# fkluger/vanishing_points_2017

Hardware: AMD Instinct MI355X
Metric: images/sec (LSD->CNN->EM) + horizon-AUC parity, YUD-shape, 1/2/4/8 GPU (higher is better)
Workload: dtype f32 (CNN: f32 operands / accumulation / results; conv1 multiply EXACT bf16 pieces of the f32 operands (three per operand) on the bf16 matrix cores; conv2-5, fc6 and fc7 multiply scaled fp16 PAIRS of the f32 operands (22 of 24 significand bits, three exact products per f32 product) on the fp16 matrix

## Files before the change

### __graft_entry__.py

```python
import os
import subprocess
import sys

ROOT = os.path.dirname(os.path.abspath(__file__))
if ROOT not in sys.path:
    sys.path.insert(0, ROOT)


def build():
    from vanishing_points_2017_amd import build as vbuild
    so = vbuild.build(verbose=True)
    sim = os.path.join(ROOT, "tests", "hostsim")
    out = os.path.join(sim, "_build")
    os.makedirs(out, exist_ok=True)
    subprocess.check_call(["g++", "-O2", "-std=c++17", "-ffp-contract=off", "-fPIC", "-shared",
                           "-Wno-unknown-pragmas", os.path.join(sim, "sim_em.cpp"), "-o",
                           os.path.join(out, "libvpk_hostsim.so")])
    subprocess.check_call(["g++", "-O2", "-std=c++17", "-ffp-contract=off", "-fPIC", "-shared",
                           os.path.join(sim, "sim_raster.cpp"), "-o", os.path.join(out, "libvpk_hostsim_raster.so")])
    subprocess.check_call(["g++", "-O2", "-std=c++17", "-Wall", "-Werror", "-fPIC", "-shared",
                           os.path.join(sim, "sim_cnn_plan.cpp"), "-o", os.path.join(out, "libvpk_hostsim_cnn_plan.so")])
    odir = os.path.join(ROOT, "oracle", "_build")
    os.makedirs(odir, exist_ok=True)
    subprocess.check_call(["gcc", "-O2", "-fPIC", "-shared", "-ffp-contract=off", "-fno-builtin",
                           os.path.join(ROOT, "oracle", "_fma.c"), "-o", os.path.join(odir, "libvpkfma.so"), "-lm"])
    import vanishing_points_2017_amd
    from vanishing_points_2017_amd import _lib
    lib = _lib.load()
    missing = [s for s in _lib.EXPORTS if not hasattr(lib, s)]
    if missing:
        raise RuntimeError("libvpk.so lacks symbols: %s" % missing)
    print("built", so)


def smoke():
    import numpy as np
    import torch
    assert torch.cuda.is_available(), "smoke() needs cuda:0"
    from vanishing_points_2017_amd import synth, vp_localisation
    from oracle import em_numpy
    from oracle import agg_raster
    from vanishing_points_2017_amd import sphere_mapping
    sc = synth.make_scene(4242, 90, 3)
    ln = sc["l"]
    sc["sphere_image"] = sphere_mapping.sphere_line_plot(ln.copy(), 500, alpha=0.1)
    assert np.array_equal(sc["sphere_image"], agg_raster.raster(ln)), "the sphere raster differs from the oracle"
    got = vp_localisation.expectation_maximisation(sc["l"].copy(), sc["lp"].copy(), sc["cnn_response"],
                                                   sphere_image=sc["sphere_image"])
    ref = em_numpy.expectation_maximisation(sc["l"].copy(), sc["lp"].copy(), sc["cnn_response"].copy(),
                                            sphere_image=sc["sphere_image"])
    assert np.array_equal(got["vp_assoc"], ref["vp_assoc"]), "line->VP assignments differ from the oracle"
    assert np.abs(got["vp"] - ref["vp"]).max() < 1e-4
    from oracle import cnn_torch
    from vanishing_points_2017_amd import cnn
    w, mean = cnn.synthetic_weights(0), cnn.synthetic_mean(0)
    sphere = sc["sphere_image"][None]
    want = cnn_torch.forward(w, mean, sphere)
    net = cnn.Net(w, mean)
    err = []
    for alg in (4, 2):
        net.set_algorithm(alg)
        err.append(float(np.abs(net.forward(sphere) - want).max()))
    net.set_algorithm(4)
    assert max(err) <= 2e-5, "CNN response differs from the oracle: %s" % err
    print("smoke ok: raster of %d lines exact; %d VPs, %d iterations; CNN max |diff| %.1e (default: fp16 pairs) / %.1e (exact bf16 triples + Winograd f32)" % (
        ln.shape[0], got["vp"].shape[0], got["iterations"], err[0], err[1]))


if __name__ == "__main__":
    build()
    if len(sys.argv) > 1 and sys.argv[1] == "smoke":
        smoke()
```

### vanishing_points_2017_amd/csrc/cnn_dense_pieces.hpp

```cpp
#ifndef VPK_CNN_DENSE_PIECES_HPP_
#define VPK_CNN_DENSE_PIECES_HPP_

namespace {

constexpr int DP_THREADS = 512;
constexpr int DP_BM = 256, DP_BN = 128;
constexpr int DP_CHUNK = 32;
template <int NP> constexpr int DP_STAGE = NP * 2 * 4 * 1024;
constexpr int DP_NST = 3;
constexpr int DP_FOLD = 8;

struct DenseDims {
    int N, K, OC;
    int chunks, kparts, cpp;
    int mtiles, ntiles;
    float wscale, oscale;
    const int* live = nullptr;
};

template <int NP>
__global__ __launch_bounds__(256) void dense_split_kernel(const float* __restrict__ x, unsigned short* __restrict__ out, int N, int K,
                                                          int chunks, float ascale, unsigned* __restrict__ range_word, unsigned range_bit,
                                                          unsigned* __restrict__ img_range, const int* __restrict__ live) {
    const int c = blockIdx.x, nt = blockIdx.y;
    if (live) {
        N = __builtin_amdgcn_readfirstlane(*live);
        if (nt * DP_BN >= N) return;
    }
    const int j = threadIdx.x >> 6, lane = threadIdx.x & 63;
    const int n = nt * DP_BN + 32 * j + (lane & 31), h = lane >> 5;
    float v[16];
    if (n < N) {
        const f32x4v* src = reinterpret_cast<const f32x4v*>(x + (size_t)n * K + (size_t)c * DP_CHUNK + 16 * h);
#pragma unroll
        for (int q = 0; q < 4; ++q) {
            const f32x4v t = src[q];
            v[4 * q] = t[0]; v[4 * q + 1] = t[1]; v[4 * q + 2] = t[2]; v[4 * q + 3] = t[3];
        }
    } else {
#pragma unroll
        for (int e = 0; e < 16; ++e) v[e] = 0.f;
    }
    unsigned short p[3][16];
    bool bad = false;
#pragma unroll
    for (int e = 0; e < 16; ++e) {
        if (NP == 3) split3(v[e], p[0][e], p[1][e], p[2][e]);
        else split2h_guard(v[e] * ascale, p[0][e], p[1][e], bad);
    }
    if (NP == 2) {
        const unsigned long long m = __builtin_amdgcn_ballot_w64(bad);
        if (m != 0ull) {
            if (lane == 0) atomicOr(range_word, range_bit);
            if (img_range && lane < 32 && (((m | (m >> 32)) >> lane) & 1ull)) atomicOr(img_range + n, range_bit);
        }
    }
    u32x4* dst = reinterpret_cast<u32x4*>(out + ((size_t)nt * chunks + c) * (DP_STAGE<NP> / 2));
#pragma unroll
    for (int q = 0; q < NP; ++q)
#pragma unroll
        for (int s = 0; s < 2; ++s) {
            u32x4 w4;
#pragma unroll
            for (int e = 0; e < 4; ++e) w4[e] = (unsigned)p[q][8 * s + 2 * e] | ((unsigned)p[q][8 * s + 2 * e + 1] << 16);
            dst[(((q * 2 + s) * 4 + j) * 64) + lane] = w4;
        }
}

__global__ void dense_tile_weights_kernel(const float* __restrict__ w, float* __restrict__ out, int OC, int K, int chunks, long long total4) {
    const long long o4 = (long long)blockIdx.x * blockDim.x + threadIdx.x;
    if (o4 >= total4) return;
    const int kk4 = (int)(o4 % (DP_CHUNK / 4));
    const int r = (int)((o4 / (DP_CHUNK / 4)) % DP_BM);
    const long long tc = o4 / ((DP_CHUNK / 4) * DP_BM);
    const int c = (int)(tc % chunks);
    const int mt = (int)(tc / chunks);
    const int row = mt * DP_BM + r;
    f32x4v v = {0.f, 0.f, 0.f, 0.f};
    if (row < OC) v = *reinterpret_cast<const f32x4v*>(w + (size_t)row * K + (size_t)c * DP_CHUNK + 4 * kk4);
    reinterpret_cast<f32x4v*>(out)[o4] = v;
}

__global__ void dense_pair_weights_kernel(const float* __restrict__ w, unsigned short* __restrict__ out, int OC, int K, int chunks,
                                          float wscale, long long total16) {
    const long long o = (long long)blockIdx.x * blockDim.x + threadIdx.x;
    if (o >= total16) return;
    const int lane = (int)(o & 63);
    const int q = (int)((o >> 6) & 1), s_ = (int)((o >> 7) & 1), wv = (int)((o >> 8) & 7);
    const long long tc = o >> 11;
    const int c = (int)(tc % chunks), mt = (int)(tc / chunks);
    const int row = mt * DP_BM + 32 * wv + (lane & 31), h = lane >> 5;
    unsigned short p[8];
#pragma unroll
    for (int e = 0; e < 8; ++e) {
        const float x = row < OC ? w[(size_t)row * K + (size_t)c * DP_CHUNK + 16 * h + 8 * s_ + e] * wscale : 0.f;
        unsigned short h0, h1;
        split2h(x, h0, h1);
        p[e] = q == 0 ? h0 : h1;
    }
    u32x4 w4;
#pragma unroll
    for (int e = 0; e < 4; ++e) w4[e] = (unsigned)p[2 * e] | ((unsigned)p[2 * e + 1] << 16);
    reinterpret_cast<u32x4*>(out)[o] = w4;
}

__global__ __launch_bounds__(DP_THREADS, 2) void dense_pairs_kernel(DenseDims d, const unsigned short* __restrict__ wpair,
                                                                    const unsigned short* __restrict__ xfrag, float* __restrict__ part,
                                                                    int* __restrict__ item_counter, int total_items) {
    constexpr int NP = 2;
    __shared__ __attribute__((aligned(16))) unsigned char dp_lds[DP_NST * DP_STAGE<NP>];
    __shared__ int s_next[2];
    const int tid = threadIdx.x, lane = tid & 63;
    const int wave = __builtin_amdgcn_readfirstlane(tid >> 6);
    const int r31 = lane & 31, h = lane >> 5;
    const unsigned lds0 = lds_addr(dp_lds);
    typedef __attribute__((address_space(3))) const bf16x8 lds_cbf8;
    int parity = 0;
    for (int item = blockIdx.x; item < total_items;) {
        int nx = 0;
        if (tid == 0)
            asm volatile("s_nop 4\n\tglobal_atomic_add %0, %1, %2, %3 sc0" : "=v"(nx) : "v"(0), "v"(1), "s"(item_counter) : "memory");
        int t = item;
        const int mt = t % d.mtiles; t /= d.mtiles;
        const int nt = t % d.ntiles;
        const int ks = t / d.ntiles;
        const int c0 = ks * d.cpp, c1 = c0 + d.cpp < d.chunks ? c0 + d.cpp : d.chunks;
        const bf16x8* wbase = reinterpret_cast<const bf16x8*>(wpair) + ((size_t)mt * d.chunks * 8 + wave) * 256 + lane;
        const unsigned char* xsrc = reinterpret_cast<const unsigned char*>(xfrag) + (size_t)nt * d.chunks * DP_STAGE<NP>;
        bf16x8 af[3][2][NP];
        auto load_a = [&](int c, auto o_tag) {
            constexpr int o = decltype(o_tag)::value;
            const bf16x8* src = wbase + (size_t)c * (8 * 256);
#pragma unroll
            for (int s = 0; s < 2; ++s)
#pragma unroll
                for (int q = 0; q < NP; ++q) af[o][s][q] = src[(2 * s + q) * 64];
        };
        auto issue_b = [&](int c) {
            const unsigned char* src = xsrc + (size_t)c * DP_STAGE<NP>;
            const unsigned dst = lds0 + (unsigned)((c % DP_NST) * DP_STAGE<NP>);
#pragma unroll
            for (int k = 0; k < NP; ++k) {
                const int f = NP * wave + k;
                dma16((unsigned)(f * 1024 + lane * 16), src, __builtin_amdgcn_readfirstlane(dst + (unsigned)f * 1024u));
            }
        };
        f32x16 acc[4], tq[4];
#pragma unroll
        for (int j = 0; j < 4; ++j)
#pragma unroll
            for (int e = 0; e < 16; ++e) { acc[j][e] = 0.f; tq[j][e] = 0.f; }
        __builtin_amdgcn_s_barrier();
        load_a(c0, std::integral_constant<int, 0>());
        issue_b(c0);
        if (c0 + 1 < c1) { load_a(c0 + 1, std::integral_constant<int, 1>()); issue_b(c0 + 1); }
        int fold = 0;
        auto chunk = [&](auto o_tag, auto o2_tag, int c) {
            constexpr int o = decltype(o_tag)::value;
            if (c + 1 < c1) asm volatile("s_waitcnt vmcnt(%0)" ::"n"(4 + NP) : "memory"); else asm volatile("s_waitcnt vmcnt(0)" ::: "memory");
            if (c == c0 && tid == 0) { asm volatile("" : "+v"(nx)); s_next[parity] = nx + (int)gridDim.x; }
            __builtin_amdgcn_s_barrier();
            if (c + 2 < c1) { load_a(c + 2, o2_tag); issue_b(c + 2); }
            const unsigned stage = lds0 + (unsigned)((c % DP_NST) * DP_STAGE<NP> + lane * 16);
#pragma unroll
            for (int s = 0; s < 2; ++s) {
                bf16x8 bfr[4][NP];
#pragma unroll
                for (int j = 0; j < 4; ++j)
#pragma unroll
                    for (int q = 0; q < NP; ++q) bfr[j][q] = *(lds_cbf8*)(stage + (unsigned)((((q * 2 + s) * 4) + j) * 1024));
                constexpr int PA[3] = {1, 0, 0}, PB[3] = {0, 1, 0};
#pragma unroll
                for (int pr = 0; pr < 3; ++pr)
#pragma unroll
                    for (int j = 0; j < 4; ++j)
                        tq[j] = __builtin_amdgcn_mfma_f32_32x32x16_f16(__builtin_bit_cast(f16x8, af[o][s][PA[pr]]),
                                                                       __builtin_bit_cast(f16x8, bfr[j][PB[pr]]), tq[j], 0, 0, 0);
            }
            if (++fold == DP_FOLD || c + 1 == c1) {
#pragma unroll
                for (int j = 0; j < 4; ++j) {
                    acc[j] += tq[j];
#pragma unroll
                    for (int e = 0; e < 16; ++e) tq[j][e] = 0.f;
                }
                fold = 0;
            }
        };
        int c = c0;
        for (; c + 2 < c1; c += 3) {
            chunk(std::integral_constant<int, 0>(), std::integral_constant<int, 2>(), c);
            chunk(std::integral_constant<int, 1>(), std::integral_constant<int, 0>(), c + 1);
            chunk(std::integral_constant<int, 2>(), std::integral_constant<int, 1>(), c + 2);
        }
        if (c < c1) chunk(std::integral_constant<int, 0>(), std::integral_constant<int, 2>(), c);
        if (c + 1 < c1) chunk(std::integral_constant<int, 1>(), std::integral_constant<int, 0>(), c + 1);
#pragma unroll
        for (int j = 0; j < 4; ++j) {
            const int n = nt * DP_BN + 32 * j + r31;
            if (n >= d.N) continue;
            float* prow = part + ((size_t)ks * d.N + n) * d.OC + mt * DP_BM + 32 * wave + 4 * h;
#pragma unroll
            for (int q = 0; q < 4; ++q) {
                if (mt * DP_BM + 32 * wave + 8 * q >= d.OC) continue;
                f32x4v v4 = {acc[j][4 * q] * d.oscale, acc[j][4 * q + 1] * d.oscale, acc[j][4 * q + 2] * d.oscale, acc[j][4 * q + 3] * d.oscale};
                *reinterpret_cast<f32x4v*>(prow + 8 * q) = v4;
            }
        }
        item = __builtin_amdgcn_readfirstlane(s_next[parity]);
        parity ^= 1;
    }
}

template <int NP>
__global__ __launch_bounds__(DP_THREADS, 2) void dense_pieces_kernel(DenseDims d, const float* __restrict__ w,
                                                                     const unsigned short* __restrict__ xfrag, float* __restrict__ part,
                                                                     int* __restrict__ item_counter, int total_items) {
    __shared__ __attribute__((aligned(16))) unsigned char dp_lds[DP_NST * DP_STAGE<NP>];
    __shared__ int s_next[2];
// ... 127 lines not shown
```

### vanishing_points_2017_amd/csrc/cnn_norm_pool.hpp

```cpp
#ifndef VPK_CNN_NORM_POOL_HPP_
#define VPK_CNN_NORM_POOL_HPP_

namespace {

template <typename Px>
__global__ void prep_input_kernel(const Px* __restrict__ sphere, const float* __restrict__ mean,
                                  float* __restrict__ out, int plane) {
    const int p = blockIdx.x * blockDim.x + threadIdx.x;
    if (p >= plane) return;
    const size_t img = (size_t)blockIdx.y * plane;
    const int y = p / 500, x = p - y * 500;
    const int q = ((y % C1_PH) * C1_PH + (x % C1_PH)) * (C1_PW * C1_PW) + (y / C1_PH) * C1_PW + x / C1_PH;
    out[img + q] = (float)sphere[img + p] - mean[p];
}

constexpr int LRN_CCH = 16;
template <int TPH, int CB>
__global__ __launch_bounds__(256) void lrn5_pool3s2_stream_kernel(const float* __restrict__ in, float* __restrict__ out, int C,
                                                                  int H, int W, int PH, int PW, float alpha, float beta,
                                                                  int PHp, int PWp, int opad, int cgroups, const int* __restrict__ live) {
    constexpr int TR = 2 * TPH + 1, SLOTS = 4, PMAX = 256 * SLOTS;
    __shared__ float plane[2][CB][PMAX];
    const int tiles_h = (PH + TPH - 1) / TPH;
    const int th = blockIdx.x % tiles_h, cgi = (blockIdx.x / tiles_h) % cgroups, b = blockIdx.x / (tiles_h * cgroups);
// ... 80 lines not shown
                }
            out[((size_t)b * C + c) * PHp * PWp + (size_t)(ph + opad) * PWp + ox + opad] = m;
        }
        buf ^= 1;
    }
}

template <int TPH, int TPW>
__global__ __launch_bounds__(256) void lrn5_pool3s2_tiled_kernel(const float* __restrict__ in, float* __restrict__ out,
                                                                 int C, int H, int W, int PH, int PW, float alpha,
                                                                 float beta, int PHp, int PWp, int opad) {
    constexpr int CC = LRN_CCH, NPL = CC + 4;
    constexpr int TR = 2 * TPH + 1, TC = 2 * TPW + 1, NPIX = TR * TC;
    __shared__ float patch[NPL][NPIX];
    const int tiles_w = (PW + TPW - 1) / TPW, tiles_h = (PH + TPH - 1) / TPH;
    const int nch = (C + CC - 1) / CC;
    int bid = blockIdx.x;
    const int tw = bid % tiles_w; bid /= tiles_w;
    const int th = bid % tiles_h; bid /= tiles_h;
    const int ch = bid % nch;
    const int b = bid / nch;
    const int c0 = ch * CC;
    const int ph0 = th * TPH, pw0 = tw * TPW;
    const int h0 = 2 * ph0, w0 = 2 * pw0;
    const int HW = H * W;
    const float* x = in + (size_t)b * C * HW;
    constexpr int LU = 8;
    for (int e0 = threadIdx.x; e0 < NPL * NPIX; e0 += 256 * LU) {
        float v[LU];
#pragma unroll
        for (int u = 0; u < LU; ++u) {
            const int e = e0 + u * 256;
            const int pl = e / NPIX, p = e - pl * NPIX;
            const int r = p / TC, q = p - r * TC;
            const int c = c0 - 2 + pl, h = h0 + r, w = w0 + q;
            v[u] = 0.f;
            if (e < NPL * NPIX && c >= 0 && c < C && h < H && w < W) v[u] = x[(size_t)c * HW + (size_t)h * W + w];
        }
#pragma unroll
        for (int u = 0; u < LU; ++u) {
            const int e = e0 + u * 256;
            if (e < NPL * NPIX) patch[0][e] = v[u];
        }
    }
    __syncthreads();
    const float an = alpha / 5.f;
    for (int p = threadIdx.x; p < NPIX; p += 256) {
        float v0 = patch[0][p], v1 = patch[1][p], v2 = patch[2][p], v3 = patch[3][p];
#pragma unroll
        for (int k = 0; k < CC; ++k) {
            const float v4 = patch[k + 4][p];
            const float sc = 1.f + an * (v0 * v0 + v1 * v1 + v2 * v2 + v3 * v3 + v4 * v4);
            float pw_;
            if (beta == 0.75f) {
                const float r = __builtin_amdgcn_rsqf(sc);
                pw_ = r * __builtin_amdgcn_sqrtf(r);
            }
            else pw_ = powf(sc, -beta);
            patch[k + 2][p] = v2 * pw_;
            v0 = v1; v1 = v2; v2 = v3; v3 = v4;
        }
    }
    __syncthreads();
    for (int e = threadIdx.x; e < CC * TPH * TPW; e += 256) {
        const int k = e / (TPH * TPW), o = e - k * (TPH * TPW);
        const int oy = o / TPW, ox = o - oy * TPW;
        const int ph = ph0 + oy, pw = pw0 + ox, c = c0 + k;
        if (ph >= PH || pw >= PW || c >= C) continue;
        float m = -3.402823466e38f;
#pragma unroll
        for (int dy = 0; dy < 3; ++dy)
#pragma unroll
            for (int dx = 0; dx < 3; ++dx) {
                const int r = 2 * oy + dy, q = 2 * ox + dx;
                if (h0 + r < H && w0 + q < W) {
                    const float v = patch[k + 2][r * TC + q];
                    m = v > m ? v : m;
                }
            }
        out[((size_t)b * C + c) * PHp * PWp + (size_t)(ph + opad) * PWp + pw + opad] = m;
    }
}

template <int PL>
__global__ __launch_bounds__(256) void pool5_kernel(const float* __restrict__ in, float* __restrict__ out, long long planes,
                                                    const int* __restrict__ live) {
    constexpr int H = 30, W = 30, P = 15, HW = H * W, PP = P * P;
    __shared__ __attribute__((aligned(16))) float s[PL * HW];
    const long long p0 = (long long)blockIdx.x * PL;
    if (live && p0 >= (long long)*live * 256) return;
    const int np = planes - p0 < PL ? (int)(planes - p0) : PL;
    const f32x4* src = reinterpret_cast<const f32x4*>(in + p0 * HW);
    for (int q = threadIdx.x; q < np * HW / 4; q += 256) reinterpret_cast<f32x4*>(s)[q] = src[q];
    __syncthreads();
    float* dst = out + p0 * PP;
    for (int e = threadIdx.x; e < np * PP; e += 256) {
        const int pl = e / PP, o = e - pl * PP;
        const int py = o / P, px = o - py * P;
        const float* x = s + pl * HW + (2 * py) * W + 2 * px;
        const bool by = 2 * py + 2 < H, bx = 2 * px + 2 < W;
        float m = fmaxf(fmaxf(x[0], x[1]), fmaxf(x[W], x[W + 1]));
        if (bx) m = fmaxf(m, fmaxf(x[2], x[W + 2]));
        if (by) m = fmaxf(m, fmaxf(x[2 * W], x[2 * W + 1]));
        if (bx && by) m = fmaxf(m, x[2 * W + 2]);
        dst[e] = m;
    }
}

__global__ void unpad_kernel(const float* __restrict__ in, float* __restrict__ out, long long planes, int H, int W,
                             int Hp, int Wp, int pad) {
    long long idx = (long long)blockIdx.x * blockDim.x + threadIdx.x;
    if (idx >= planes * H * W) return;
    const int w = (int)(idx % W), hh = (int)((idx / W) % H);
    const long long pl = idx / ((long long)W * H);
    out[idx] = in[((size_t)pl * Hp + hh + pad) * Wp + w + pad];
}

}
#endif
```

### vanishing_points_2017_amd/csrc/cnn_plan.hpp

```cpp
#ifndef VPK_CNN_PLAN_HPP_
#define VPK_CNN_PLAN_HPP_

#include "../../include/vpk.h"

struct CnnConfig {
    int precision = 0;
    int split_variant = 0;
    int algorithm = 4;
    int fusion = 3;
    int conv1_group = 4;
    int dense_presplit = 1;
    bool profiling = false;
};

inline void cnn_config_set_precision(CnnConfig& c, int mode) {
    c.precision = mode ? 1 : 0;
    c.split_variant = mode > 1 ? mode - 1 : 0;
}

enum class Conv1Impl { GEMM, DIRECT_F32, GEMM_FUSED, PIECES3, PIECES2 };
enum class ConvImpl { DMA_F32, SPLIT_GEMM, WINOGRAD, PIECES3, PIECES2 };
enum class DenseImpl { DMA_F32, PIECES3, PIECES2_STREAMED, PIECES2_PRESPLIT };

struct ConvStage {
    ConvImpl impl = ConvImpl::DMA_F32;
    int split_tiling = 0;
    bool chained_in = false;
    bool chained_out = false;
    bool needs_to_planes = false;
    bool writes_next_planes = false;
};

struct CnnPlan {
    int err = VPK_OK;
    const char* msg = nullptr;
    bool prep_input = false;
    Conv1Impl conv1 = Conv1Impl::PIECES3;
    bool conv1_hands_planes = false;
    ConvStage conv[4];
    bool norm2_planes = false;
    bool norm2_hands_planes = false;
    DenseImpl fc[3] = {DenseImpl::DMA_F32, DenseImpl::DMA_F32, DenseImpl::DMA_F32};
};

inline CnnPlan cnn_resolve_plan(const CnnConfig& c, int tap, bool f32_images, bool device_counted) {
    CnnPlan p;
    const bool f32_mfma = c.precision == 0;
    const bool pairs = f32_mfma && c.algorithm == 4;
    const bool triples = f32_mfma && c.algorithm >= 2 && !pairs;
    const bool wino = f32_mfma && c.algorithm >= 1;
    const bool split = c.precision == 1;

    if (tap == 0 || c.fusion == 0) p.conv1 = Conv1Impl::GEMM;
    else if (c.fusion == 1) p.conv1 = Conv1Impl::DIRECT_F32;
    else if (c.fusion == 2) p.conv1 = Conv1Impl::GEMM_FUSED;
    else p.conv1 = c.fusion == 4 ? Conv1Impl::PIECES2 : Conv1Impl::PIECES3;
    p.prep_input = p.conv1 == Conv1Impl::GEMM || p.conv1 == Conv1Impl::GEMM_FUSED;
    const bool conv1_pieces = p.conv1 == Conv1Impl::PIECES3 || p.conv1 == Conv1Impl::PIECES2;
    p.conv1_hands_planes = conv1_pieces && pairs && tap != 1;
    if (f32_images && p.conv1 == Conv1Impl::PIECES2) {
        p.err = VPK_ERR_STATE;
        p.msg = "vpk_cnn_forward_f32: vpk_cnn_set_fusion(4) takes uint8 rasters only";
    }

    const ConvImpl pieces = pairs ? ConvImpl::PIECES2 : ConvImpl::PIECES3;
    const ConvImpl other = split ? ConvImpl::SPLIT_GEMM : (wino ? ConvImpl::WINOGRAD : ConvImpl::DMA_F32);
    const bool pieces35 = pairs || (triples && c.algorithm == 3);
    p.conv[0].impl = pairs || triples ? pieces : other;
    p.conv[1].impl = pieces35 ? pieces : other;
    p.conv[2].impl = pairs ? pieces : other;
    p.conv[3].impl = pieces35 ? pieces : other;
    p.norm2_planes = pairs;
    p.norm2_hands_planes = pairs && tap != 3;
    p.conv[1].writes_next_planes = pairs && tap != 4;
    p.conv[2].writes_next_planes = pairs && tap != 5;
    p.conv[0].needs_to_planes = (pairs || triples) && !p.conv1_hands_planes;
    p.conv[1].needs_to_planes = pieces35 && !p.norm2_hands_planes;
    p.conv[2].needs_to_planes = pairs && !p.conv[1].writes_next_planes;
    p.conv[3].needs_to_planes = pieces35 && !p.conv[2].writes_next_planes;
    const bool chain = split && tap != 4 && tap != 5;
    p.conv[1].chained_out = p.conv[2].chained_in = p.conv[2].chained_out = p.conv[3].chained_in = chain;
    for (int i = 0; i < 4; ++i) p.conv[i].split_tiling = c.split_variant == 0 ? (i <= 1 ? 1 : 0) : c.split_variant - 1;

    const DenseImpl dense2 = c.dense_presplit ? DenseImpl::PIECES2_PRESPLIT : DenseImpl::PIECES2_STREAMED;
    if (pairs) p.fc[0] = p.fc[1] = dense2;
    else if (triples) p.fc[0] = DenseImpl::PIECES3;

    if (device_counted) {
        const bool counted = p.conv1 == Conv1Impl::PIECES3 && p.conv[0].impl == ConvImpl::PIECES3 &&
                             p.conv[1].impl == ConvImpl::WINOGRAD && p.conv[2].impl == ConvImpl::WINOGRAD &&
                             p.conv[3].impl == ConvImpl::WINOGRAD && !p.norm2_planes && p.fc[0] == DenseImpl::PIECES3 &&
                             p.fc[1] == DenseImpl::DMA_F32 && p.fc[2] == DenseImpl::DMA_F32 && tap < 0 && !c.profiling;
        if (!counted) {
            p.err = VPK_ERR_STATE;
            p.msg = "run_forward: a device-counted pass runs algorithm 2 with the default conv1, untapped";
        }
    }
    return p;
}

#endif
```

### vanishing_points_2017_amd/csrc/vpk_cnn.hip

```cpp
#include "vpk_internal.hpp"

#include <stdlib.h>
#include <string.h>
#include <type_traits>
#include <vector>

#include "cnn_plan.hpp"
#include "cnn_topology.hpp"
#include "cnn_gemm_f32.hpp"
#include "cnn_conv1_direct.hpp"
#include "cnn_norm_pool.hpp"

namespace {

#include "cnn_split_gemm.hpp"
#include "cnn_pairs.hpp"
#include "cnn_conv1_pieces.hpp"
#include "cnn_conv_pieces.hpp"
#include "cnn_norm_pool_planes.hpp"
#include "cnn_dense_pieces.hpp"
#include "cnn_winograd.hpp"

struct Layer {
    ConvDims d;
// ... 243 lines not shown
                               S->L[1].wino, S->L[1].bias, dst, ctr + 1, total);
            return;
        }
        WinoDims wd = S->L[li].wd;
        wd.tiles = batch * WG_TILES_PER_IMAGE;
        const int total = wd.groups * wd.ocblocks * ((wd.tiles + WG_TB - 1) / WG_TB);
        hipLaunchKernelGGL(conv3x3_winograd_kernel, dim3((unsigned)std::min(total, h->num_cu)), dim3(WG_THREADS), 0, st, wd, src,
                           S->L[li].wino, S->L[li].bias, dst, ctr + li, total, live);
    };
    auto to_p6 = [&](int li, bool pairs, const float* src, unsigned short* dst) {
        const ConvDims& d = S->L[li].d;
        const int C = d.IC * d.groups;
        if (pairs) hipLaunchKernelGGL(to_planes_kernel<2>, dim3((unsigned)d.Hp, (unsigned)(C / 16), (unsigned)batch), dim3(256), 0, st, src, dst, C, d.Hp, d.Wp,
                                      S->L[li].ascale, fc.range_word, 1u << li, fc.img_range, live);
        else hipLaunchKernelGGL(to_planes_kernel<3>, dim3((unsigned)d.Hp, (unsigned)(C / 16), (unsigned)batch), dim3(256), 0, st, src, dst, C, d.Hp, d.Wp, 1.f,
                                fc.range_word, 0u, nullptr, live);
    };
    auto conv_pieces = [&](int li, bool pairs, const unsigned short* src6, float* dst, unsigned short* planes_next) {
        PieceDims pd = pairs ? S->L[li].pdh : S->L[li].pd;
        pd.B = batch;
        if (planes_next) { const PieceDims& nx = S->L[li + 1].pdh; pd.o_cgtot = nx.CGtot; pd.o_Hp = nx.Hp; pd.o_Wp = nx.Wp; pd.o_pad = 1; pd.o_ascale = S->L[li + 1].ascale; }
        pd.range_word = fc.range_word; pd.range_bit = 1u << (li + 1); pd.img_range = fc.img_range; pd.live = live;
        if (pairs) pd.oscale = 1.f / (S->L[li].hscale * S->L[li].ascale);
        constexpr int nb = 4;
        const int tile_rows = pairs && li == 3 ? 2 * nb : nb;
        pd.rtiles = (pd.OH + tile_rows - 1) / tile_rows;
        const int total = pd.groups * batch * pd.rtiles * pd.ctiles * pd.mtiles;
        const unsigned blocks = (unsigned)std::min(total, 2 * h->num_cu);
        auto go = [&](auto kernel) {
            hipLaunchKernelGGL(kernel, dim3(blocks), dim3(CP_THREADS), 0, st, pd, src6, pairs ? S->L[li].whalf : S->L[li].wsplit, S->L[li].bias,
                               dst, planes_next, ctr + li, total);
        };
        if (pairs) { if (li == 1) go(conv_pieces_kernel<5, nb, 2, 1>); else if (li == 3) go(conv_pieces_kernel<3, nb, 2, 2>); else go(conv_pieces_kernel<3, nb, 2, 1>); }
        else { if (li == 1) go(conv_pieces_kernel<5, nb, 3, 1>); else go(conv_pieces_kernel<3, nb, 3, 1>); }
    };
    auto conv_stage = [&](int li, const float* src, float* dst, unsigned short* planes, unsigned short* planes_next,
                          const unsigned short* split_in, unsigned short* split_out) {
        const ConvStage& cs = plan.conv[li - 1];
        const bool pairs = cs.impl == ConvImpl::PIECES2;
        switch (cs.impl) {
        case ConvImpl::PIECES3:
        case ConvImpl::PIECES2:
            if (cs.needs_to_planes) to_p6(li, pairs, src, planes);
            conv_pieces(li, pairs, planes, dst, cs.writes_next_planes ? planes_next : nullptr);
            break;
        case ConvImpl::SPLIT_GEMM:
            conv_split(li, cs.split_tiling, src, cs.chained_in ? split_in : nullptr, cs.chained_out ? (void*)split_out : (void*)dst, cs.chained_out);
            break;
        case ConvImpl::WINOGRAD:
            conv_wino(li, src, dst);
            break;
        case ConvImpl::DMA_F32:
            if (li == 3) launch_dma(h, conv_gemm_dma_kernel<1, 4, 3, 1, false>, dims(3), 96, src, S->L[3], dst, 1, ctr + 3);
            else launch_dma(h, conv_gemm_dma_kernel<2, 2, 2, 2, false>, dims(li), 128, src, S->L[li], dst, 1, ctr + li);
            break;
        }
    };
    unsigned short* p6_2 = reinterpret_cast<unsigned short*>(R[R_P6_2]);
    unsigned short* p6_3 = reinterpret_cast<unsigned short*>(R[R_P6_3]);
    unsigned short* p6_5 = reinterpret_cast<unsigned short*>(R[R_P6_5]);
    unsigned short* s4 = reinterpret_cast<unsigned short*>(R[R_SPLIT4]);
    unsigned short* s5 = reinterpret_cast<unsigned short*>(R[R_SPLIT5]);
    conv_stage(1, R[R_POOL1], R[R_CONV2], p6_2, nullptr, nullptr, nullptr);
    mark(1);
    if ((rc = tapcopy(2, R[R_CONV2], A_CONV2))) return rc;
    if (plan.norm2_planes)
        hipLaunchKernelGGL((lrn5_pool3s2_planes_kernel<6>), dim3((unsigned)(batch * 5 * 8)), dim3(256), 0, st, R[R_CONV2], R[R_POOL2],
                           plan.norm2_hands_planes ? p6_3 : nullptr, 256, 61, 61, 30, 30, 1e-4f, 32, 32, 1, 8,
                           S->L[2].ascale, fc.range_word, 1u << 2, fc.img_range);
    else
        hipLaunchKernelGGL((lrn5_pool3s2_stream_kernel<6, 4>), dim3((unsigned)(batch * 5 * 8)), dim3(256), 0, st, R[R_CONV2], R[R_POOL2],
                           256, 61, 61, 30, 30, 1e-4f, 0.75f, 32, 32, 1, 8, live);
    mark(2);
    tapunpad(3, R[R_POOL2], 256, 30, 30, 1);
    conv_stage(2, R[R_POOL2], R[R_CONV3], p6_3, p6_5, nullptr, s4);
    mark(1);
    tapunpad(4, R[R_CONV3], 384, 30, 30, 1);
    conv_stage(3, R[R_CONV3], R[R_CONV4], p6_5, p6_3, s4, s5);
    mark(1);
    tapunpad(5, R[R_CONV4], 384, 30, 30, 1);
    conv_stage(4, R[R_CONV4], R[R_CONV5], plan.conv[2].writes_next_planes ? p6_3 : p6_5, nullptr, s5, nullptr);
    mark(1);
    if ((rc = tapcopy(6, R[R_CONV5], A_CONV5))) return rc;
    hipLaunchKernelGGL((pool5_kernel<8>), dim3((unsigned)(((long long)batch * 256 + 7) / 8)), dim3(256), 0, st, R[R_CONV5], R[R_POOL5],
                       (long long)batch * 256, live);
    mark(1);
    if ((rc = tapcopy(7, R[R_POOL5], A_POOL5))) return rc;

    float* fc_in = R[R_POOL5];
    float* fc_out = R[R_FCA];
    for (int li = 5; li < 8; ++li) {
        ConvDims d = dims(li);
        const DenseImpl impl = plan.fc[li - 5];
        if (impl == DenseImpl::DMA_F32) {
            launch_dma(h, conv_gemm_dma_kernel<2, 2, 2, 2, true>, d, 128, fc_in, S->L[li], R[R_PART], 1, ctr + li, 3, live);
        } else {
            const bool pairs = impl != DenseImpl::PIECES3;
            DenseDims dd;
            dd.N = batch; dd.K = d.K; dd.OC = d.OC; dd.chunks = d.K / DP_CHUNK;
            dd.kparts = li == 5 ? 45 : 16;
            dd.cpp = dd.chunks / dd.kparts;
            dd.mtiles = (d.OC + DP_BM - 1) / DP_BM; dd.ntiles = (batch + DP_BN - 1) / DP_BN;
            dd.wscale = pairs ? S->L[li].hscale : 1.f;
            dd.live = live;
            dd.oscale = pairs ? 1.f / (S->L[li].hscale * S->L[li].ascale) : 1.f;
            const size_t need = (size_t)dd.ntiles * (TOPO[5].IC / DP_CHUNK) * DP_STAGE<3>;
            if ((rc = vpk_reserve(h, (void**)&S->xfrag, &S->xfrag_bytes, need, "hipMalloc(dense input fragments)"))) return rc;
            const int total = dd.mtiles * dd.ntiles * dd.kparts;
            const dim3 split_grid((unsigned)dd.chunks, (unsigned)dd.ntiles), grid((unsigned)std::min(total, h->num_cu));
            if (pairs)
                hipLaunchKernelGGL(dense_split_kernel<2>, split_grid, dim3(256), 0, st, fc_in, S->xfrag, batch,
                                   d.K, dd.chunks, S->L[li].ascale, fc.range_word, 1u << li, fc.img_range, nullptr);
            else
                hipLaunchKernelGGL(dense_split_kernel<3>, split_grid, dim3(256), 0, st, fc_in, S->xfrag, batch,
                                   d.K, dd.chunks, 1.f, fc.range_word, 0u, nullptr, live);
            switch (impl) {
            case DenseImpl::PIECES2_PRESPLIT:
                hipLaunchKernelGGL(dense_pairs_kernel, grid, dim3(DP_THREADS), 0, st, dd, S->L[li].wpair, S->xfrag, R[R_PART], ctr + li, total);
                break;
            case DenseImpl::PIECES2_STREAMED:
                hipLaunchKernelGGL(dense_pieces_kernel<2>, grid, dim3(DP_THREADS), 0, st, dd, S->L[li].wraw, S->xfrag, R[R_PART], ctr + li, total);
                break;
            default:
                hipLaunchKernelGGL(dense_pieces_kernel<3>, grid, dim3(DP_THREADS), 0, st, dd, S->L[li].wraw, S->xfrag, R[R_PART], ctr + li, total);
                break;
            }
            d.ksplit = dd.kparts;
        }
        const long long tot = (long long)d.N * d.OC;
        float* dst = li == 7 ? out : fc_out;
        float* pre = (li == 7 && tap == 10) ? tap_out : nullptr;
        hipLaunchKernelGGL(splitk_reduce_kernel, dim3(ew_blocks(tot)), dim3(256), 0, st, R[R_PART], S->L[li].bias, d.ksplit,
                           d.N, d.OC, li == 7 ? 2 : 1, dst, pre, live);
        mark(1);
        if (li == 5 && (rc = tapcopy(8, fc_out, A_FC6))) return rc;
        if (li == 6 && (rc = tapcopy(9, fc_out, A_FC7))) return rc;
        fc_in = fc_out;
        fc_out = (li == 5) ? R[R_FCB] : R[R_FCA];
    }
    if (cfg.profiling) {
        S->ev_valid = (evi == 14);
        if (S->ev_valid) ++S->ev_pass;
    }
    VPK_HIP(h, hipGetLastError());
    return VPK_OK;
}

}
#include "cnn_calibrate.hpp"
#include "cnn_range_policy.hpp"

namespace {

struct ScopedDeviceBuffer {
    void* p = nullptr;
    ~ScopedDeviceBuffer() { if (p) (void)hipFree(p); }
};

template <typename T>
int upload(vpk_handle* h, T** dst, const T* src, size_t n) {
    VPK_HIP(h, hipMalloc((void**)dst, n * sizeof(T)));
    VPK_HIP(h, hipMemcpy(*dst, src, n * sizeof(T), hipMemcpyHostToDevice));
    return VPK_OK;
}

int load_model(vpk_handle* h, const float* const blobs[16], const float* mean) {
    vpk_cnn_state* S = h->cnn;
    int rc;
    if ((rc = upload(h, &S->mean, mean, (size_t)500 * 500))) return rc;
    if (const char* e = getenv("VPK_CONV1_GROUP")) { const int v = atoi(e); if (v >= 1 && v <= 64) S->cfg.conv1_group = v; }
    if (const char* e = getenv("VPK_DENSE_PRESPLIT")) S->cfg.dense_presplit = atoi(e) != 0;
    for (int li = 0; li < 8; ++li) {
        const Topo& t = TOPO[li];
        const float* w = blobs[2 * li];
        Layer& l = S->L[li];
        ConvDims& d = l.d;
        d.B = 0; d.IC = t.IC; d.Hp = t.H + 2 * t.P; d.Wp = t.W + 2 * t.P; d.OC = t.OC; d.OH = t.OH; d.OW = t.OW; d.groups = t.G;
        d.OHp = t.OH + 2 * t.OP; d.OWp = t.OW + 2 * t.OP; d.opad = t.OP;
        if (li == 0) { d.IC = C1_PH * C1_PH; d.Hp = C1_PW; d.Wp = C1_PW; }
        d.K = t.IC * t.KH * t.KH;
        d.Kp = (d.K + BK - 1) / BK * BK;
        d.Mp = (t.OC + t.BM - 1) / t.BM * t.BM;
        d.N = 0;
        d.ksplit = KSPLIT[li];
        d.relu = 1;
        const size_t w_floats = (size_t)t.G * t.OC * d.K;
        const size_t p_floats = (size_t)t.G * d.Kp * d.Mp;
        {
            ScopedDeviceBuffer rawbuf;
            VPK_HIP(h, hipMalloc(&rawbuf.p, w_floats * sizeof(float)));
            const float* raw = static_cast<const float*>(rawbuf.p);
            VPK_HIP(h, hipMemcpy(rawbuf.p, w, w_floats * sizeof(float), hipMemcpyHostToDevice));
            VPK_HIP(h, hipMalloc((void**)&l.wp, p_floats * sizeof(float)));
            hipLaunchKernelGGL(pack_weights_kernel, dim3((unsigned)((p_floats + 255) / 256)), dim3(256), 0, h->stream, raw,
                               l.wp, t.G, t.OC, d.K, d.Kp, d.Mp);
            VPK_HIP(h, hipStreamSynchronize(h->stream));
            if (li == 5 || li == 6) {
                const int chunks = d.K / DP_CHUNK, mtiles = (t.OC + DP_BM - 1) / DP_BM;
                const long long total4 = (long long)mtiles * chunks * DP_BM * (DP_CHUNK / 4);
                VPK_HIP(h, hipMalloc((void**)&l.wraw, (size_t)total4 * 16));
                hipLaunchKernelGGL(dense_tile_weights_kernel, dim3((unsigned)((total4 + 255) / 256)), dim3(256), 0, h->stream, raw, l.wraw, t.OC, d.K,
                                   chunks, total4);
                VPK_HIP(h, hipStreamSynchronize(h->stream));
                l.hscale = weight_scale_pow2(w, w_floats);
                const long long total16 = (long long)mtiles * chunks * 8 * 2 * 2 * 64;
                VPK_HIP(h, hipMalloc((void**)&l.wpair, (size_t)total16 * 16));
                hipLaunchKernelGGL(dense_pair_weights_kernel, dim3((unsigned)((total16 + 255) / 256)), dim3(256), 0, h->stream, raw, l.wpair, t.OC,
                                   d.K, chunks, l.hscale, total16);
                VPK_HIP(h, hipStreamSynchronize(h->stream));
            }
        }
        if (li < 5) {
            std::vector<unsigned> tab(d.Kp, 0u);
            for (int k = 0; k < d.K; ++k) {
                int ic = k / (t.KH * t.KH), r = k % (t.KH * t.KH), kh = r / t.KH, kw = r % t.KH;
                if (li == 0)
// ... 291 lines not shown
```

Measured before the change: 23270.

## Fuse pool5 and fc6 reduce with fp16-pair fragment packing for dense layers

Pool5 now writes the fc6 input directly as scaled fp16 pair fragments in the dense kernel's layout. The fc6 split-k reduce likewise applies bias and ReLU and emits fc7's input fragments directly. This removes the separate float round trips and dense_split launches for fc6 and fc7 on the default path. Weight fragment loads in the dense kernel also become nontemporal. The trade-off is extra index arithmetic and scattered 16-byte stores, and taps 7/8 fall back to the old path.

```diff
diff --git a/__graft_entry__.py b/__graft_entry__.py
--- a/__graft_entry__.py
+++ b/__graft_entry__.py
@@ -20,6 +20,8 @@
                            os.path.join(sim, "sim_raster.cpp"), "-o", os.path.join(out, "libvpk_hostsim_raster.so")])
     subprocess.check_call(["g++", "-O2", "-std=c++17", "-Wall", "-Werror", "-fPIC", "-shared",
                            os.path.join(sim, "sim_cnn_plan.cpp"), "-o", os.path.join(out, "libvpk_hostsim_cnn_plan.so")])
+    subprocess.check_call(["g++", "-O2", "-std=c++17", "-Wall", "-Werror", "-fPIC", "-shared",
+                           os.path.join(sim, "sim_cnn_dense_tail.cpp"), "-o", os.path.join(out, "libvpk_hostsim_cnn_dense_tail.so")])
     odir = os.path.join(ROOT, "oracle", "_build")
     os.makedirs(odir, exist_ok=True)
     subprocess.check_call(["gcc", "-O2", "-fPIC", "-shared", "-ffp-contract=off", "-fno-builtin",
diff --git a/vanishing_points_2017_amd/csrc/cnn_dense_pieces.hpp b/vanishing_points_2017_amd/csrc/cnn_dense_pieces.hpp
--- a/vanishing_points_2017_amd/csrc/cnn_dense_pieces.hpp
+++ b/vanishing_points_2017_amd/csrc/cnn_dense_pieces.hpp
@@ -65,6 +65,78 @@
             for (int e = 0; e < 4; ++e) w4[e] = (unsigned)p[q][8 * s + 2 * e] | ((unsigned)p[q][8 * s + 2 * e + 1] << 16);
             dst[(((q * 2 + s) * 4 + j) * 64) + lane] = w4;
         }
+}
+
+__device__ __forceinline__ size_t dense_frag_word(int n, int k, int q, int chunks) {
+    const int c = k / DP_CHUNK, kk = k % DP_CHUNK, h = kk >> 4, s = (kk >> 3) & 1;
+    const int nt = n / DP_BN, j = (n % DP_BN) >> 5, lane = (n & 31) + 32 * h;
+    return ((size_t)nt * chunks + c) * (DP_STAGE<2> / 16) + (size_t)(((q * 2 + s) * 4 + j) * 64 + lane);
+}
+
+constexpr int P5F_PL = 8, P5F_GROUPS = 256 / P5F_PL, P5F_K = P5F_PL * P5_PP;
+__global__ __launch_bounds__(256) void pool5_frags_kernel(const float* __restrict__ in, unsigned short* __restrict__ out, int N, float ascale,
+                                                          unsigned* __restrict__ range_word, unsigned range_bit,
+                                                          unsigned* __restrict__ img_range) {
+    static_assert(P5F_K % 8 == 0 && (256 * P5_PP) % DP_CHUNK == 0, "whole fragment words per workgroup, whole chunks per image");
+    constexpr int chunks = 256 * P5_PP / DP_CHUNK;
+    __shared__ __attribute__((aligned(16))) float s[P5F_PL * P5_HW];
+    __shared__ __attribute__((aligned(16))) unsigned short hp[2][P5F_K];
+    const int b = blockIdx.x, u = (b >> 6) * 8 + (b & 7);
+    const int pg = u % P5F_GROUPS, n = (u / P5F_GROUPS) * 8 + ((b >> 3) & 7);
+    u32x4* dst = reinterpret_cast<u32x4*>(out);
+    const int k0 = pg * P5F_K;
+    if (n >= N) {
+        const u32x4 z = {0u, 0u, 0u, 0u};
+        for (int w = threadIdx.x; w < 2 * (P5F_K / 8); w += 256) {
+            const int q = w / (P5F_K / 8), g = w - q * (P5F_K / 8);
+            dst[dense_frag_word(n, k0 + 8 * g, q, chunks)] = z;
+        }
+        return;
+    }
+    const f32x4* src = reinterpret_cast<const f32x4*>(in + ((size_t)n * 256 + (size_t)pg * P5F_PL) * P5_HW);
+    for (int q = threadIdx.x; q < P5F_PL * P5_HW / 4; q += 256) reinterpret_cast<f32x4*>(s)[q] = src[q];
+    __syncthreads();
+    bool bad = false;
+    for (int e = threadIdx.x; e < P5F_K; e += 256) {
+        const int pl = e / P5_PP, o = e - pl * P5_PP;
+        split2h_guard(pool5_window(s + pl * P5_HW, o) * ascale, hp[0][e], hp[1][e], bad);
+    }
+    range_report(bad, range_word, range_bit, img_range ? img_range + n : nullptr);
+    __syncthreads();
+    for (int w = threadIdx.x; w < 2 * (P5F_K / 8); w += 256) {
+        const int q = w / (P5F_K / 8), g = w - q * (P5F_K / 8);
+        dst[dense_frag_word(n, k0 + 8 * g, q, chunks)] = reinterpret_cast<const u32x4*>(hp[q])[g];
+    }
+}
+
+__global__ __launch_bounds__(256) void splitk_reduce_frags_kernel(const float* __restrict__ part, const float* __restrict__ bias, int ksplit,
+                                                                  int N, int OC, unsigned short* __restrict__ out, float ascale,
+                                                                  unsigned* __restrict__ range_word, unsigned range_bit,
+                                                                  unsigned* __restrict__ img_range) {
+    const int per = OC / 4;
+    const long long t = (long long)blockIdx.x * 256 + threadIdx.x;
+    const int n = (int)(t / per), m = 4 * (int)(t % per);
+    f32x4v v = {0.f, 0.f, 0.f, 0.f};
+    if (n < N) {
+        const f32x4v* p = reinterpret_cast<const f32x4v*>(part + (size_t)n * OC + m);
+        const size_t stride = (size_t)N * OC / 4;
+#pragma unroll 15
+        for (int s = 0; s < ksplit; ++s) v += p[s * stride];
+        v += *reinterpret_cast<const f32x4v*>(bias + m);
+#pragma unroll
+        for (int e = 0; e < 4; ++e) v[e] = v[e] > 0.f ? v[e] : 0.f;
+    }
+    unsigned short h0[4], h1[4];
+    bool bad = false;
+#pragma unroll
+    for (int e = 0; e < 4; ++e) split2h_guard(v[e] * ascale, h0[e], h1[e], bad);
+    range_report(bad, range_word, range_bit, img_range && n < N ? img_range + n : nullptr);
+    const unsigned hi[2] = {(unsigned)h0[0] | ((unsigned)h0[1] << 16), (unsigned)h0[2] | ((unsigned)h0[3] << 16)};
+    const unsigned lo[2] = {(unsigned)h1[0] | ((unsigned)h1[1] << 16), (unsigned)h1[2] | ((unsigned)h1[3] << 16)};
+    const bool odd = threadIdx.x & 1;
+    const unsigned r0 = (unsigned)__shfl_xor((int)(odd ? hi[0] : lo[0]), 1), r1 = (unsigned)__shfl_xor((int)(odd ? hi[1] : lo[1]), 1);
+    const u32x4 w4 = odd ? u32x4{r0, r1, lo[0], lo[1]} : u32x4{hi[0], hi[1], r0, r1};
+    reinterpret_cast<u32x4*>(out)[dense_frag_word(n, odd ? m - 4 : m, odd ? 1 : 0, OC / DP_CHUNK)] = w4;
 }
 
 __global__ void dense_tile_weights_kernel(const float* __restrict__ w, float* __restrict__ out, int OC, int K, int chunks, long long total4) {
@@ -134,7 +206,7 @@
 #pragma unroll
             for (int s = 0; s < 2; ++s)
 #pragma unroll
-                for (int q = 0; q < NP; ++q) af[o][s][q] = src[(2 * s + q) * 64];
+                for (int q = 0; q < NP; ++q) af[o][s][q] = __builtin_nontemporal_load(&src[(2 * s + q) * 64]);
         };
         auto issue_b = [&](int c) {
             const unsigned char* src = xsrc + (size_t)c * DP_STAGE<NP>;
diff --git a/vanishing_points_2017_amd/csrc/cnn_norm_pool.hpp b/vanishing_points_2017_amd/csrc/cnn_norm_pool.hpp
--- a/vanishing_points_2017_amd/csrc/cnn_norm_pool.hpp
+++ b/vanishing_points_2017_amd/csrc/cnn_norm_pool.hpp
@@ -186,10 +186,24 @@
     }
 }
 
+constexpr int P5_H = 30, P5_W = 30, P5_P = 15, P5_HW = P5_H * P5_W, P5_PP = P5_P * P5_P;
+
+__device__ __forceinline__ float pool5_window(const float* __restrict__ plane, int o) {
+    constexpr int H = P5_H, W = P5_W, P = P5_P;
+    const int py = o / P, px = o - py * P;
+    const float* x = plane + (2 * py) * W + 2 * px;
+    const bool by = 2 * py + 2 < H, bx = 2 * px + 2 < W;
+    float m = fmaxf(fmaxf(x[0], x[1]), fmaxf(x[W], x[W + 1]));
+    if (bx) m = fmaxf(m, fmaxf(x[2], x[W + 2]));
+    if (by) m = fmaxf(m, fmaxf(x[2 * W], x[2 * W + 1]));
+    if (bx && by) m = fmaxf(m, x[2 * W + 2]);
+    return m;
+}
+
 template <int PL>
 __global__ __launch_bounds__(256) void pool5_kernel(const float* __restrict__ in, float* __restrict__ out, long long planes,
                                                     const int* __restrict__ live) {
-    constexpr int H = 30, W = 30, P = 15, HW = H * W, PP = P * P;
+    constexpr int HW = P5_HW, PP = P5_PP;
     __shared__ __attribute__((aligned(16))) float s[PL * HW];
     const long long p0 = (long long)blockIdx.x * PL;
     if (live && p0 >= (long long)*live * 256) return;
@@ -200,14 +214,7 @@
     float* dst = out + p0 * PP;
     for (int e = threadIdx.x; e < np * PP; e += 256) {
         const int pl = e / PP, o = e - pl * PP;
-        const int py = o / P, px = o - py * P;
-        const float* x = s + pl * HW + (2 * py) * W + 2 * px;
-        const bool by = 2 * py + 2 < H, bx = 2 * px + 2 < W;
-        float m = fmaxf(fmaxf(x[0], x[1]), fmaxf(x[W], x[W + 1]));
-        if (bx) m = fmaxf(m, fmaxf(x[2], x[W + 2]));
-        if (by) m = fmaxf(m, fmaxf(x[2 * W], x[2 * W + 1]));
-        if (bx && by) m = fmaxf(m, x[2 * W + 2]);
-        dst[e] = m;
+        dst[e] = pool5_window(s + pl * HW, o);
     }
 }
 
diff --git a/vanishing_points_2017_amd/csrc/cnn_plan.hpp b/vanishing_points_2017_amd/csrc/cnn_plan.hpp
--- a/vanishing_points_2017_amd/csrc/cnn_plan.hpp
+++ b/vanishing_points_2017_amd/csrc/cnn_plan.hpp
@@ -41,6 +41,8 @@
     bool norm2_planes = false;
     bool norm2_hands_planes = false;
     DenseImpl fc[3] = {DenseImpl::DMA_F32, DenseImpl::DMA_F32, DenseImpl::DMA_F32};
+    bool pool5_hands_frags = false;
+    bool fc6_hands_frags = false;
 };
 
 inline CnnPlan cnn_resolve_plan(const CnnConfig& c, int tap, bool f32_images, bool device_counted) {
@@ -85,6 +87,9 @@
     const DenseImpl dense2 = c.dense_presplit ? DenseImpl::PIECES2_PRESPLIT : DenseImpl::PIECES2_STREAMED;
     if (pairs) p.fc[0] = p.fc[1] = dense2;
     else if (triples) p.fc[0] = DenseImpl::PIECES3;
+    const bool default_arithmetic = pairs && c.fusion == 3;
+    p.pool5_hands_frags = default_arithmetic && tap != 7;
+    p.fc6_hands_frags = default_arithmetic && tap != 8;
 
     if (device_counted) {
         const bool counted = p.conv1 == Conv1Impl::PIECES3 && p.conv[0].impl == ConvImpl::PIECES3 &&
diff --git a/vanishing_points_2017_amd/csrc/vpk_cnn.hip b/vanishing_points_2017_amd/csrc/vpk_cnn.hip
--- a/vanishing_points_2017_amd/csrc/vpk_cnn.hip
+++ b/vanishing_points_2017_amd/csrc/vpk_cnn.hip
@@ -349,8 +349,18 @@
     conv_stage(4, R[R_CONV4], R[R_CONV5], plan.conv[2].writes_next_planes ? p6_3 : p6_5, nullptr, s5, nullptr);
     mark(1);
     if ((rc = tapcopy(6, R[R_CONV5], A_CONV5))) return rc;
-    hipLaunchKernelGGL((pool5_kernel<8>), dim3((unsigned)(((long long)batch * 256 + 7) / 8)), dim3(256), 0, st, R[R_CONV5], R[R_POOL5],
-                       (long long)batch * 256, live);
+    const int dense_ntiles = (batch + DP_BN - 1) / DP_BN;
+    auto reserve_xfrag = [&]() {
+        const size_t need = (size_t)dense_ntiles * (TOPO[5].IC / DP_CHUNK) * DP_STAGE<3>;
+        return vpk_reserve(h, (void**)&S->xfrag, &S->xfrag_bytes, need, "hipMalloc(dense input fragments)");
+    };
+    if (plan.pool5_hands_frags) {
+        if ((rc = reserve_xfrag())) return rc;
+        hipLaunchKernelGGL(pool5_frags_kernel, dim3((unsigned)(dense_ntiles * DP_BN * P5F_GROUPS)), dim3(256), 0, st, R[R_CONV5], S->xfrag,
+                           batch, S->L[5].ascale, fc.range_word, 1u << 5, fc.img_range);
+    } else
+        hipLaunchKernelGGL((pool5_kernel<8>), dim3((unsigned)(((long long)batch * 256 + 7) / 8)), dim3(256), 0, st, R[R_CONV5], R[R_POOL5],
+                           (long long)batch * 256, live);
     mark(1);
     if ((rc = tapcopy(7, R[R_POOL5], A_POOL5))) return rc;
 
@@ -367,18 +377,18 @@
             dd.N = batch; dd.K = d.K; dd.OC = d.OC; dd.chunks = d.K / DP_CHUNK;
             dd.kparts = li == 5 ? 45 : 16;
             dd.cpp = dd.chunks / dd.kparts;
-            dd.mtiles = (d.OC + DP_BM - 1) / DP_BM; dd.ntiles = (batch + DP_BN - 1) / DP_BN;
+            dd.mtiles = (d.OC + DP_BM - 1) / DP_BM; dd.ntiles = dense_ntiles;
             dd.wscale = pairs ? S->L[li].hscale : 1.f;
             dd.live = live;
             dd.oscale = pairs ? 1.f / (S->L[li].hscale * S->L[li].ascale) : 1.f;
-            const size_t need = (size_t)dd.ntiles * (TOPO[5].IC / DP_CHUNK) * DP_STAGE<3>;
-            if ((rc = vpk_reserve(h, (void**)&S->xfrag, &S->xfrag_bytes, need, "hipMalloc(dense input fragments)"))) return rc;
+            if ((rc = reserve_xfrag())) return rc;
             const int total = dd.mtiles * dd.ntiles * dd.kparts;
             const dim3 split_grid((unsigned)dd.chunks, (unsigned)dd.ntiles), grid((unsigned)std::min(total, h->num_cu));
-            if (pairs)
+            const bool handed = (li == 5 && plan.pool5_hands_frags) || (li == 6 && plan.fc6_hands_frags);
+            if (!handed && pairs)
                 hipLaunchKernelGGL(dense_split_kernel<2>, split_grid, dim3(256), 0, st, fc_in, S->xfrag, batch,
                                    d.K, dd.chunks, S->L[li].ascale, fc.range_word, 1u << li, fc.img_range, nullptr);
-            else
+            else if (!handed)
                 hipLaunchKernelGGL(dense_split_kernel<3>, split_grid, dim3(256), 0, st, fc_in, S->xfrag, batch,
                                    d.K, dd.chunks, 1.f, fc.range_word, 0u, nullptr, live);
             switch (impl) {
@@ -397,8 +407,12 @@
         const long long tot = (long long)d.N * d.OC;
         float* dst = li == 7 ? out : fc_out;
         float* pre = (li == 7 && tap == 10) ? tap_out : nullptr;
-        hipLaunchKernelGGL(splitk_reduce_kernel, dim3(ew_blocks(tot)), dim3(256), 0, st, R[R_PART], S->L[li].bias, d.ksplit,
-                           d.N, d.OC, li == 7 ? 2 : 1, dst, pre, live);
+        if (li == 5 && plan.fc6_hands_frags)
+            hipLaunchKernelGGL(splitk_reduce_frags_kernel, dim3((unsigned)((long long)dense_ntiles * DP_BN * (d.OC / 4) / 256)), dim3(256), 0, st,
+                               R[R_PART], S->L[5].bias, d.ksplit, batch, d.OC, S->xfrag, S->L[6].ascale, fc.range_word, 1u << 6, fc.img_range);
+        else
+            hipLaunchKernelGGL(splitk_reduce_kernel, dim3(ew_blocks(tot)), dim3(256), 0, st, R[R_PART], S->L[li].bias, d.ksplit,
+                               d.N, d.OC, li == 7 ? 2 : 1, dst, pre, live);
         mark(1);
         if (li == 5 && (rc = tapcopy(8, fc_out, A_FC6))) return rc;
         if (li == 6 && (rc = tapcopy(9, fc_out, A_FC7))) return rc;
```

New measurement: 23440, median of 3. About the same (+0.7%).
